# logv/sybil

Hardware: AMD Instinct MI355X
Metric: rows scanned/sec (1B-row x 32-int-col synthetic table, 3 ANDed int-range filters, group-by 2 cols, count/sum/avg/stddev of 2 cols) (higher is better)
Workload: dtype int64

## Files before the change

sybil_amd/csrc/planner.cpp:

```cpp
#include <math.h>
#include <stdlib.h>
#include <string.h>

#include <algorithm>

#include "engine.h"
#include "hll.h"
#include "re2lite.h"

namespace sybl {

static inline int64_t round_up(int64_t x, int64_t m) { return (x + m - 1) / m * m; }


struct HostFilterFold {
    bool has_range = false;
    int64_t lo = INT64_MIN, hi = INT64_MAX;
    std::vector<int64_t> neq;
    bool has_mask = false;
    std::vector<uint8_t> mask;
    std::vector<std::pair<int32_t, int32_t>> setp;
};

static void setup_buckets(int64_t info_min, int64_t info_max, int64_t hist_bucket, int64_t *bucket_size,
                          int64_t *num_buckets, int64_t *n_values) {
    int64_t size = info_max - info_min;
    int64_t nb = 1000;
    int64_t bs = size / nb;
    if (hist_bucket > 0) bs = hist_bucket;
    if (bs == 0) {
        if (size < 100) {
            bs = 1;
            nb = size;
        } else {
            bs = size / 100;
            nb = size / bs;
        }
    }
    nb += 1;
    *bucket_size = bs;
    *num_buckets = nb;
    *n_values = nb + 1;
}


static bool should_scan_block(const Table *t, const sybl_query_desc *d, int64_t b) {
    for (int i = 0; i < d->n_filters; i++) {
        const sybl_filter &f = d->filters[i];
        const Column *c = t->find(f.col);
        if (!c || c->type != SYBL_INT_VAL) continue;
        if (f.op != SYBL_OP_GT && f.op != SYBL_OP_LT && f.op != SYBL_OP_EQ) continue;
        if (c->blk_pop[(size_t)b] == 0) return false;
        int64_t mn = c->blk_min[(size_t)b], mx = c->blk_max[(size_t)b], v = f.int_value;
        if (f.op == SYBL_OP_GT && !(mn > v) && !(mx > v)) return false;
        if (f.op == SYBL_OP_LT && !(mn < v) && !(mx < v)) return false;
        if (f.op == SYBL_OP_EQ && (mn > v || mx < v)) return false;
    }
    return true;
}

constexpr int kEffWeightCol = -2;
constexpr int kRankColBase = -100;
static inline Column *slot_column(const Table *t, const Query *q, int ci) {
    if (ci <= kRankColBase) return t->cols[(size_t)(kRankColBase - ci)]->rank_col.get();
    return ci == kEffWeightCol ? q->eff_weight.get() : t->cols[(size_t)ci].get();
}

static bool fill_packed(Table *t, Query *q, const std::vector<int> &slot_col, FastPlan &FP, int nf, int ng, int na) {
    const ScanPlan &P = q->plan;
    if (env("SYBL_NO_PACKED")) return false;
    if (P.n_cells >= (1 << 24)) return false;
    for (int c = 0; c < nf; c++) {
        const __int128 umax = ((__int128)1 << (8 * FP.fwid[c])) - 1;
        const __int128 L = (__int128)FP.lo[c] - FP.fbase[c], H = (__int128)FP.hi[c] - FP.fbase[c];
        if (H < 0 || L > umax || L > H) {
            FP.plo[c] = 1;
            FP.phi[c] = 0;
        } else {
            FP.plo[c] = (uint32_t)(L < 0 ? 0 : L);
            FP.phi[c] = (uint32_t)(H > umax ? umax : H);
        }
        FP.npneq[c] = 0;
        for (int k = 0; k < FP.nneq[c]; k++) {
            const __int128 off = (__int128)FP.neq[c][k] - FP.fbase[c];
            if (off >= 0 && off <= umax) FP.pneq[c][FP.npneq[c]++] = (uint32_t)off;
        }
    }
    {
        double pass = 1.0;
        for (int c = 0; c < nf; c++) {
            const Column *col = nullptr;
            for (auto &cp : t->cols) {
                if (cp->d_data == (const void *)FP.fcol[c]) col = cp.get();
                if (cp->rank_col && cp->rank_col->d_data == (const void *)FP.fcol[c]) col = cp->rank_col.get();
            }
            if (FP.plo[c] > FP.phi[c]) {
                pass = 0.0;
            } else if (col && col->n_pop > 0 && col->exact_max >= col->vbase && !FP.fmask[c]) {
                const double top = (double)((__int128)col->exact_max - (__int128)col->vbase);
                const double hi = std::min((double)FP.phi[c], top), lo = (double)FP.plo[c];
                pass *= hi >= lo ? std::min(1.0, (hi - lo + 1.0) / (top + 1.0)) : 0.0;
            }
        }
        q->late_estimate = pass;
        FP.late = nf > 0 && pass < 0.005 ? 1 : 0;
        if (const char *e = env("SYBL_LATE_PATH")) FP.late = atoi(e) != 0;
    }
    for (int c = 0; c < ng; c++) FP.gdoff[c] = (uint32_t)((uint64_t)FP.gbase[c] - (uint64_t)FP.gmin[c]);
    for (int c = 0; c < na; c++) {
        const __int128 L = (__int128)FP.info_min[c] - FP.abase[c], H = (__int128)FP.max10[c] - FP.abase[c];
        const __int128 umax = ((__int128)1 << 32) - 1;
        if (H < 0 || L > umax || L > H) {
            FP.alo[c] = 1;
            FP.ahi[c] = 0;
        } else {
            FP.alo[c] = (uint32_t)(L < 0 ? 0 : L);
            FP.ahi[c] = (uint32_t)(H > umax ? umax : H);
        }
    }
    const double shave = 1.0 - 1.0 / (double)((int64_t)1 << 40);
    for (int c = 0; c < na; c++) {
        FP.adoff[c] = (uint32_t)((uint64_t)FP.abase[c] - (uint64_t)FP.hmin[c]);
        FP.pinv_bucket[c] = FP.bucket_size[c] ? (1.0 / (double)FP.bucket_size[c]) * shave : 0.0;
    }
    if (q->time_mode) {
        const SlotDesc &ts = P.slot[P.time_slot];
        const Column *tc = slot_column(t, q, slot_col[(size_t)P.time_slot]);
        if (P.tb_big_div || P.time_bucket >= ((int64_t)1 << 32)) return false;
        if (tc->n_pop > 0 && tc->exact_min < 0) return false;
        const __int128 t0 = (__int128)P.tb_min * P.time_bucket;
        const __int128 off = (__int128)ts.vbase - t0;
        const __int128 top = tc->n_pop > 0 ? (__int128)tc->exact_max - t0 : off;
        if (off < 0 || top >= ((__int128)1 << 32)) return false;
        FP.tdoff = (uint32_t)off;
        FP.pinv_time = (1.0 / (double)P.time_bucket) * shave;
    }
    return true;
}

#define FF_REJECT(...)                                                                                  \
    do {                                                                                                \
        if (env("SYBL_PLAN_TRACE")) fprintf(stderr, "fast path: rejected at planner.cpp:%d\n", __LINE__); \
        return __VA_ARGS__;                                                                             \
    } while (0)

static bool fill_fast_columns(Table *t, Query *q, const std::vector<int> &slot_col, FastPlan &FP, int *pnf, int *png,
                              int *pna, bool *any_max, bool *all_max, bool allow_gen, bool *gen, bool *packed = nullptr,
                              int max_groups = kFastTemplatedG, int max_aggs = kFastTemplatedA, bool part = false) {
    const ScanPlan &P = q->plan;
    memset(&FP, 0, sizeof(FP));
    int nf = 0, ng = 0, na = 0;
    *gen = false;
    bool any_packed = false, all_narrow = true;
    bool heavy = false;
    bool nul_needed = false;
    if (packed) *packed = false;
    for (size_t s = 0; s < slot_col.size(); s++) {
        const SlotDesc &sd = P.slot[s];
        if (sd.flags == 0 && q->pre_n_slots > 0) continue;
        const Column *c = slot_column(t, q, slot_col[s]);
        bool plain = c->type == SYBL_INT_VAL && !c->d_valid && !c->has_missing;
        any_packed = any_packed || c->packed();
        all_narrow = all_narrow && c->elem <= 4;
        if (!plain) {
            if (!allow_gen) FF_REJECT(false);
            uint32_t r2 = sd.flags & (kSlotFilter | kSlotGroup | kSlotAgg | kSlotTime);
            bool str_ok = c->type == SYBL_STR_VAL && (r2 == kSlotGroup || r2 == kSlotIdMask || r2 == (kSlotGroup | kSlotIdMask));
            if (c->type != SYBL_INT_VAL && !str_ok) FF_REJECT(false);
            *gen = true;
            if (c->d_valid || c->has_missing || (sd.flags & kSlotIdMask)) nul_needed = true;
        }
        uint32_t roles = sd.flags & (kSlotFilter | kSlotGroup | kSlotAgg);
        if (sd.flags & (kSlotSet | kSlotDict)) FF_REJECT(false);
        if ((sd.flags & kSlotNeq) && (!allow_gen || c->type != SYBL_INT_VAL)) FF_REJECT(false);
        if ((sd.flags & kSlotIdMask) && !allow_gen) FF_REJECT(false);
        if ((sd.flags & kSlotWeight) && (roles != 0 || (sd.flags & kSlotTime) || !allow_gen)) FF_REJECT(false);
// ... 1224 lines not shown
    std::vector<Segment> runs;
    bool quiet = false;

    int64_t max_lane_rows() const {
        if (q->dyn) return (int64_t)q->piece_cap * q->piece_tiles * kPackedRows;
        int64_t lane_rows = 0;
        for (int w = 0; w < q->n_wg; w++) {
            int64_t mine = 0;
            for (int32_t si = q->wg_seg_begin[(size_t)w]; si < q->wg_seg_begin[(size_t)w + 1]; si++)
                mine += (q->segs[(size_t)si].n + kPackedTileRows - 1) / kPackedTileRows * kPackedRows;
            lane_rows = std::max(lane_rows, mine);
        }
        return lane_rows;
    }

    void plan_count_packing() {
        FastPlan &FP = q->fplan;
        FP.cshift = 0;
        if (!q->fast || !q->fast_packed || q->fast_packed_n || q->part_hist || FP.nul || q->fast_na < 1 || env("SYBL_NO_CPACK")) return;
        if (q->fast_mode != kFastAvg && q->fast_mode != kFastAvgMax) return;
        const int64_t lane_rows = max_lane_rows();
        const unsigned __int128 slot_rows = (unsigned __int128)std::max<int64_t>(lane_rows, 1) * (unsigned __int128)(kWgThreads >> P.rep_shift);
        const Column *c = t->cols[(size_t)q->aggs[0].col].get();
        unsigned __int128 umax = c->elem >= 4 ? 0xFFFFFFFFull : c->elem == 2 ? 0xFFFFull : 0xFFull;
        if (c->n_pop > 0 && c->exact_max >= c->vbase) umax = std::min<unsigned __int128>(umax, (unsigned __int128)((__int128)c->exact_max - (__int128)c->vbase));
        auto bits = [](unsigned __int128 x) {
            int b = 0;
            while (x) b++, x >>= 1;
            return b;
        };
        const int sum_bits = std::max(1, bits(umax * slot_rows)), count_bits = bits(slot_rows);
        if (sum_bits + count_bits <= 64 && sum_bits < 63) FP.cshift = sum_bits;
        if (env("SYBL_PLAN_TRACE") && !quiet)
            fprintf(stderr, "count packing: cshift=%d sum_bits=%d count_bits=%d slot_rows=%lld\n", (int)FP.cshift, sum_bits, count_bits, (long long)slot_rows);
    }

    void plan_lean() {
        FastPlan &FP = q->fplan;
        FP.lean = 0;
        FP.lds_sum_fields = 0;
        if (!q->fast || !q->fast_packed || q->fast_packed_n || q->part_hist || FP.nul || q->fast_na < 1 || env("SYBL_NO_LEAN")) return;
        if (q->fast_mode != kFastMoments && q->fast_mode != kFastHist) return;
        const int na = q->fast_na;
        bool digits = !P.windowed, mul24 = true;
        for (size_t g = 0; g < q->groups.size() && digits; g++) {
            const int ci = q->groups[g].col;
            const Column *c = ci >= 0 ? t->cols[(size_t)ci].get() : nullptr;
            if (!c || c->type != SYBL_INT_VAL || c->n_pop <= 0 || q->groups[g].dict || q->groups[g].rank) {
                digits = false;
                break;
            }
            const __int128 lo = (__int128)c->exact_min - (__int128)FP.gmin[g], hi = (__int128)c->exact_max - (__int128)FP.gmin[g];
            digits = lo >= 0 && hi < (__int128)FP.gcard[g];
        }
        for (int a = 0; a < na; a++) {
            const Column *c = t->cols[(size_t)q->aggs[(size_t)a].col].get();
            if (FP.bucket_size[a] >= (1u << 24)) mul24 = false;
            if (c->n_pop > 0) {
                const __int128 lo = (__int128)c->exact_min - (__int128)FP.hmin[a], hi = (__int128)c->exact_max - (__int128)FP.hmin[a];
                if (lo < 0 || hi >= ((__int128)1 << 24)) mul24 = false;
            }
        }
        if (digits && mul24) FP.lean |= (int32_t)kLeanProved;
        if (q->fast_mode != kFastMoments) {
            if (env("SYBL_PLAN_TRACE") && !quiet) fprintf(stderr, "lean hist: proved=%d digits=%d mul24=%d\n", (FP.lean & (int32_t)kLeanProved) ? 1 : 0, (int)digits, (int)mul24);
            return;
        }
        const int words_now = P.n_sum_fields, words_lean = lean_sum_fields(na);
        bool shape = P.n_max_fields == 0 && P.n_sum_fields == 1 + 3 * na && FP.f_samples < 0 && FP.hist_lds == 0;
        for (int a = 0; a < na; a++) shape = shape && FP.f_sum[a] > 0 && FP.f_sb[a] > 0 && FP.f_sb2[a] > 0 && FP.f_cnt[a] < 0 && FP.f_pop[a] < 0 && FP.f_out[a] < 0;
        int rs = 0, cshift = 0;
        unsigned __int128 slot_rows = 0;
        uint64_t umax[kFastMaxA] = {0}, bmax[kFastMaxA] = {0};
        if (shape) {
            int64_t budget = kLdsBudgetBytes;
            if (!P.windowed)
                if (const char *e = env("SYBL_REP_BUDGET_KB")) budget = std::min<int64_t>(kLdsBudgetBytes, std::max<int64_t>(1, atoll(e)) * 1024);
            const int64_t bytes = (int64_t)words_lean * P.lds_cells * 8;
            while (rs < 6 && (bytes << (rs + 1)) <= budget) rs++;
            slot_rows = (unsigned __int128)std::max<int64_t>(max_lane_rows(), 1) * (unsigned __int128)(kWgThreads >> rs);
            for (int a = 0; a < na; a++) {
                const Column *c = t->cols[(size_t)q->aggs[(size_t)a].col].get();
                unsigned __int128 u = c->elem >= 4 ? 0xFFFFFFFFull : c->elem == 2 ? 0xFFFFull : 0xFFull;
                if (c->n_pop > 0 && c->exact_max >= c->vbase) u = std::min<unsigned __int128>(u, (unsigned __int128)((__int128)c->exact_max - (__int128)c->vbase));
                umax[a] = (uint64_t)u;
                bmax[a] = (uint64_t)std::max(FP.n_values[a] - 1, 0);
            }
            cshift = lean_moments_fit(na, umax, bmax, slot_rows);
        }
        if (cshift) {
            FP.lean |= (int32_t)kLeanMoments;
            FP.lds_sum_fields = words_lean;
            FP.cshift = cshift;
            P.rep_shift = rs;
            FP.rep_shift = rs;
            q->lds_bytes = ((size_t)words_lean * (size_t)P.lds_cells * 8) << rs;
        }
        if (env("SYBL_PLAN_TRACE") && !quiet) {
            fprintf(stderr, "lean moments: lean=%d proved=%d digits=%d mul24=%d cshift=%d count_bits=%d", cshift ? 1 : 0, (FP.lean & (int32_t)kLeanProved) ? 1 : 0,
                    (int)digits, (int)mul24, cshift, lean_bits(slot_rows));
            for (int a = 0; a < na && shape; a++)
                fprintf(stderr, " s%d_bits=%d b%d_bits=%d q%d_bits=%d", a, lean_bits((unsigned __int128)umax[a] * slot_rows), a,
                        lean_bits((unsigned __int128)bmax[a] * slot_rows), a, lean_bits((unsigned __int128)bmax[a] * bmax[a] * slot_rows));
            fprintf(stderr, " slot_rows=%lld tried_replicas=%d words=%d replicas=%d\n", (long long)slot_rows, 1 << rs, cshift ? words_lean : words_now,
                    1 << P.rep_shift);
        }
    }

    void plan_dynamic() {
        FastPlan &FP = q->fplan;
        const int32_t rep_shift0 = P.rep_shift, fp_rep_shift0 = FP.rep_shift;
        const size_t lds_bytes0 = q->lds_bytes;
        auto proofs = [&](bool dyn, bool silent) {
            P.rep_shift = rep_shift0;
            FP.rep_shift = fp_rep_shift0;
            q->lds_bytes = lds_bytes0;
// ... 520 lines not shown
```

sybil_amd/csrc/scan_fast.h:

```cpp
#pragma once
#include <hip/hip_runtime.h>
#include <stdint.h>

#include "plan.h"
#include "pieces.h"
#include "outlog.h"
#include "wg_header.h"

namespace sybl {

constexpr int kFastMaxF = 4, kFastMaxG = 4, kFastMaxA = 4;
constexpr int kFastTemplatedG = 2, kFastTemplatedA = 2;

enum FastMode : int {
    kFastAvg = 0,
    kFastAvgMax = 1,
    kFastMoments = 2,
    kFastHist = 3,
    kFastModes = 4,
};

struct FastPlan {
    const int64_t *fcol[kFastMaxF];
    const int64_t *gcol[kFastMaxG];
// ... 8 lines not shown
    int32_t n_values[kFastMaxA];
    int32_t f_sum[kFastMaxA], f_sb[kFastMaxA], f_sb2[kFastMaxA], m_max[kFastMaxA];
    int32_t m_nmin[kFastMaxA];
    int32_t ext_general;
    int64_t hist_agg_off[kFastMaxA];
    int64_t hist_off, hist_stride;
    int32_t n_cells, n_sum_fields, n_max_fields, rep_shift;
    const int64_t *tcol;
    int64_t time_bucket, tb_min;
    double inv_time_bucket;
    int32_t n_tb, tb_stride;
    int32_t windowed, lds_cells;
    int32_t hist_lds;
    int32_t lean;
    const uint32_t *fvalid[kFastMaxF], *gvalid[kFastMaxG], *avalid[kFastMaxA], *tvalid;
    int32_t gmissing[kFastMaxG], gvalues[kFastMaxG];
    int64_t gstride64[kFastMaxG], gmissing64[kFastMaxG], gvalues64[kFastMaxG], tb_stride64;
    const uint32_t *fmask[kFastMaxF];
    int32_t fmask_bits[kFastMaxF];
    int32_t nneq[kFastMaxF], npneq[kFastMaxF];
    int64_t neq[kFastMaxF][kMaxNeq];
    uint32_t pneq[kFastMaxF][kMaxNeq];
    int32_t f_cnt[kFastMaxA], f_pop[kFastMaxA], f_smp[kFastMaxA], f_out[kFastMaxA];
    int64_t info_min[kFastMaxA], max10[kFastMaxA];
    const int64_t *wcol;
    int32_t f_samples;
    int32_t cshift;
    int32_t fwid[kFastMaxF], gwid[kFastMaxG], awid[kFastMaxA], twid, wwid;
    int64_t fbase[kFastMaxF], gbase[kFastMaxG], abase[kFastMaxA], tbase, wbase;
    uint32_t plo[kFastMaxF], phi[kFastMaxF];
    uint32_t gdoff[kFastMaxG];
    uint32_t adoff[kFastMaxA];
    uint32_t tdoff;
    int32_t late;
    double pinv_bucket[kFastMaxA], pinv_time;
    uint32_t alo[kFastMaxA], ahi[kFastMaxA];
    int32_t nul;
    int32_t lds_sum_fields;
    const int32_t *wg_cell_base;
    const uint32_t *xvalid;
    int64_t *out_log;
    int64_t out_cap;
    int64_t *sum_out, *max_out, *ws_sum, *ws_max;
    const Segment *segs;
    const int32_t *wg_seg_begin;
    unsigned long long *wg_clock;
    int32_t dyn, n_pieces, piece_cap;
    const Piece *pieces;
    uint32_t *piece_queue;
    const uint32_t *fword;
    int32_t fshift[kFastMaxF], fbits[kFastMaxF];
    const uint32_t *kword;
    int32_t gshift[kFastMaxG], gbits[kFastMaxG], kashift, kabits;
};

hipError_t launch_scan_fast(const FastPlan &P, int nf, int ng, int na, int mode, bool time, bool gen, int n_wg,
                            size_t lds_bytes, hipStream_t st);

inline bool fast_plan_has_narrow(const FastPlan &P, bool aggs) {
    bool any = P.twid == 3 || P.wwid == 3 || (aggs && P.kword != nullptr);
    for (int c = 0; c < kFastMaxF; c++) any = any || P.fwid[c] == 3;
    for (int c = 0; c < kFastMaxG; c++) any = any || P.gwid[c] == 3;
    for (int c = 0; aggs && c < kFastMaxA; c++) any = any || P.awid[c] == 3;
    return any;
}

constexpr uint32_t kLeanMoments = 1u, kLeanProved = 2u;
constexpr int lean_sum_fields(int na) { return na + (na + 1) / 2 + na; }
constexpr int lean_bits(unsigned __int128 x) {
    int b = 0;
    while (x) b++, x >>= 1;
    return b;
}
constexpr int lean_moments_fit(int na, const uint64_t *umax, const uint64_t *bmax, unsigned __int128 slot_rows) {
    const unsigned __int128 one = 1;
    if (na < 1 || slot_rows < 1 || slot_rows >= (one << 63)) return 0;
    const int sum_bits = lean_bits((unsigned __int128)umax[0] * slot_rows) < 1 ? 1 : lean_bits((unsigned __int128)umax[0] * slot_rows);
    const int count_bits = lean_bits(slot_rows);
    if (!(sum_bits + count_bits <= 64 && sum_bits < 63)) return 0;
    const int shift = sum_bits < 32 ? 32 : sum_bits;
    if (shift + count_bits > 64) return 0;
    for (int c = 0; c < na; c++) {
        if (umax[c] >= (one << 32) || bmax[c] >= (one << 24)) return 0;
        if (c >= 1 && lean_bits((unsigned __int128)umax[c] * slot_rows) > 64) return 0;
        if (lean_bits((unsigned __int128)bmax[c] * bmax[c] * slot_rows) > 64) return 0;
        if ((unsigned __int128)bmax[c] * slot_rows >= (one << 32)) return 0;
    }
    return shift;
}
namespace lean_check {
constexpr uint64_t kU0[1] = {0}, kBfit[1] = {65535}, kBnot[1] = {65536};
static_assert(lean_moments_fit(1, kU0, kBfit, 65537) == 32, "sum(b) up to 2^32 - 1 fits a dword");
static_assert(lean_moments_fit(1, kU0, kBnot, 65536) == 0, "sum(b) of 2^32 does not");
constexpr uint64_t kU64[1] = {((uint64_t)1 << 23) - 1}, kU65[1] = {(uint64_t)1 << 23}, kB0[1] = {0};
static_assert(lean_moments_fit(1, kU64, kB0, (unsigned __int128)1 << 20) == 43, "64 bits of sum and count fit");
static_assert(lean_moments_fit(1, kU65, kB0, (unsigned __int128)1 << 20) == 0, "65 bits do not");
}

constexpr int kPartCells = 64;
constexpr int kPartCellBits = 6;
constexpr int kBucketBits = 10;
constexpr int kRecValueBits = 26;
constexpr int kMaxParts = 1024;
constexpr int kEmitMaxBins = 1024;
constexpr uint32_t kEmitChunk = 16;
constexpr uint32_t kEmitQueue = 32;
// ... 1072 lines not shown
```

sybil_amd/csrc/scan_packed.h:

```cpp
#pragma once
#include "narrow3.h"
#include "fword.h"
#include "scan_fast.h"

namespace sybl {

constexpr int kPackedRows = 4;
constexpr int kPackedTileRows = kWgThreads * kPackedRows;

hipError_t launch_scan_packed(const FastPlan &P, int nf, int ng, int na, int mode, bool time, int n_wg, size_t lds_bytes,
                              hipStream_t st);
hipError_t launch_emit_packed(const EmitPlan &E, int nf, int ng, int na, int n_wg, hipStream_t st);
hipError_t launch_count_packed_nf0(const EmitPlan &E, int ng, int n_wg, hipStream_t st);
hipError_t launch_count_packed_nf1(const EmitPlan &E, int ng, int n_wg, hipStream_t st);
hipError_t launch_count_packed_nf2(const EmitPlan &E, int ng, int n_wg, hipStream_t st);
hipError_t launch_count_packed_nf3(const EmitPlan &E, int ng, int n_wg, hipStream_t st);
hipError_t launch_count_packed_nf4(const EmitPlan &E, int ng, int n_wg, hipStream_t st);
hipError_t launch_emit_packed_nf0(const EmitPlan &E, int ng, int na, int n_wg, hipStream_t st);
hipError_t launch_emit_packed_nf1(const EmitPlan &E, int ng, int na, int n_wg, hipStream_t st);
hipError_t launch_emit_packed_nf2(const EmitPlan &E, int ng, int na, int n_wg, hipStream_t st);
hipError_t launch_emit_packed_nf3(const EmitPlan &E, int ng, int na, int n_wg, hipStream_t st);
hipError_t launch_emit_packed_nf4(const EmitPlan &E, int ng, int na, int n_wg, hipStream_t st);
hipError_t launch_scan_packed_nf0(const FastPlan &P, int ng, int na, int mode, bool time, int n_wg, size_t lds, hipStream_t st);
hipError_t launch_scan_packed_nf1(const FastPlan &P, int ng, int na, int mode, bool time, int n_wg, size_t lds, hipStream_t st);
// ... 122 lines not shown
__device__ __forceinline__ void packed_issue_ring(const FastPlan &P, const PackedBases<NF, NG, NA> &B, uint32_t r, uint32_t n,
                                                  PackedRaw<NF> &f, PackedRaw<NG> &g, PackedRaw<NA> &a, PackedRaw<1> &t) {
    const uint32_t r0 = __builtin_amdgcn_readfirstlane(r);
    const uint32_t lane_row = r - r0;
    const uint32_t rows = r0 < n ? (n - r0 < 64u * kPackedRows ? (n - r0 + kPackedRows - 1) & ~(uint32_t)(kPackedRows - 1) : 64u * kPackedRows) : 0u;
    const uint32_t base_row = rows ? r0 : 0u;
    auto issue = [&](const uint8_t *col, int width, pu32x4 &raw) {
        const uint32_t w = (uint32_t)width;
        const __amdgpu_buffer_rsrc_t rsrc =
            __builtin_amdgcn_make_buffer_rsrc((void *)(col + (size_t)(base_row * w)), 0, (int)(rows * w), (int)kBufferRsrcWord3);
        raw = __builtin_amdgcn_raw_buffer_load_b128(rsrc, (int)(__umul24(lane_row, w)), 0, 2);
    };
    if (TIME) issue(B.t, P.twid, t.v[0]);
#pragma unroll
    for (int c = 0; c < NF; c++) issue(B.f[c], P.fwid[c], f.v[c]);
#pragma unroll
    for (int c = 0; c < NG; c++) {
        if (G1) {
            const __amdgpu_buffer_rsrc_t rsrc = __builtin_amdgcn_make_buffer_rsrc((void *)(B.g[c] + (size_t)base_row), 0, (int)rows, (int)kBufferRsrcWord3);
            g.v[c].x = __builtin_amdgcn_raw_buffer_load_b32(rsrc, (int)lane_row, 0, 2);
        } else {
            issue(B.g[c], P.gwid[c], g.v[c]);
        }
    }
#pragma unroll
    for (int c = 0; c < NA; c++) issue(B.a[c], P.awid[c], a.v[c]);
}

constexpr int packed_depth(int) { return 1; }

template <int NF, int NG, int NA, bool TIME, bool G1, bool NUL, bool FRESH = false>
__device__ __forceinline__ void packed_decode_all(const FastPlan &P0, const PackedRaw<NF> &rf, const PackedRaw<NG> &rg,
                                                  const PackedRaw<NA> &ra, const PackedRaw<1> &rt, PackedTile<NF> &f,
                                                  PackedTile<NG> &g, PackedTile<NA> &a, PackedTile<1> &t, uint32_t bit0) {
    const FastPlan &P = plan_fresh<FRESH>(P0);
    if (NUL) {
        if (TIME) t.pop[0] = (rt.pw[0] >> bit0) & 0xFu;
#pragma unroll
        for (int c = 0; c < NF; c++) f.pop[c] = (rf.pw[c] >> bit0) & 0xFu;
#pragma unroll
        for (int c = 0; c < NG; c++) g.pop[c] = (rg.pw[c] >> bit0) & 0xFu;
#pragma unroll
        for (int c = 0; c < NA; c++) a.pop[c] = (ra.pw[c] >> bit0) & 0xFu;
    }
    if (TIME) packed_decode(P.twid, rt.v[0], t.u[0]);
#pragma unroll
    for (int c = 0; c < NF; c++) packed_decode(P.fwid[c], rf.v[c], f.u[c]);
#pragma unroll
    for (int c = 0; c < NG; c++) packed_decode(G1 ? 1 : P.gwid[c], rg.v[c], g.u[c]);
#pragma unroll
    for (int c = 0; c < NA; c++) packed_decode(P.awid[c], ra.v[c], a.u[c]);
}

template <bool M24 = false>
__device__ __forceinline__ uint32_t packed_udiv(uint32_t n, uint32_t d, double inv_lo) {
    uint32_t q = (uint32_t)((double)n * inv_lo);
    if (n - (M24 ? __umul24(q, d) : q * d) >= d) q += 1;
    return q;
}

template <int NF, int NG, int NA, int MODE, bool TIME, bool NUL, bool FRESH = false, bool OUT = false, bool MAX32 = false, bool LEAN = false,
          bool PROVED = false, bool COUNTED = false, bool DERIVED = false>
__device__ __forceinline__ void packed_row(const FastPlan &P0, const PackedTile<NF> &f, const PackedTile<NG> &g,
                                           const PackedTile<NA> &a, const PackedTile<1> &t, const int r, bool pass, int64_t *lds,
                                           const FastLds &L, uint32_t &matched, uint32_t &overflow, const uint32_t xpop = 0xFu) {
    static_assert(!LEAN || (MODE == kFastMoments && !NUL && !OUT && NA >= 1), "the lean layout is the plain moments body's");
    static_assert(!PROVED || (!NUL && !OUT), "proofs cover fully populated rows");
    static_assert(!DERIVED || (!NUL && !OUT), "only a row that counts in exactly one place can have its overflow derived");
    if (NUL) pass = pass & ((xpop >> r) & 1u);
#pragma unroll
    for (int c = 0; c < NF; c++) {
        const FastPlan &P = plan_fresh<FRESH>(P0);
        const uint32_t u = f.u[c][r];
        bool ok = (u >= P.plo[c]) & (u <= P.phi[c]);
        if (NUL) {
            if (P.fmask[c]) {
                const uint32_t id = u + (uint32_t)P.fbase[c];
                ok = id < (uint32_t)P.fmask_bits[c];
                if (ok) ok = (P.fmask[c][id >> 5] >> (id & 31)) & 1u;
            }
            for (int k = 0; k < P.npneq[c]; k++) ok = ok & (u != P.pneq[c][k]);
            ok = ok & ((f.pop[c] >> r) & 1u);
        }
        pass = pass & ok;
    }
    uint32_t cell = 0;
    bool inb = true;
#pragma unroll
    for (int c = 0; c < NG; c++) {
        const FastPlan &P = plan_fresh<FRESH>(P0);
        const uint32_t d = g.u[c][r] + P.gdoff[c];
        if (NUL) {
            const bool p = (g.pop[c] >> r) & 1u;
            inb = inb & (p ? d < (uint32_t)P.gvalues[c] : P.gmissing[c] >= 0);
            cell += p ? __umul24(d, (uint32_t)P.gstride[c]) : (uint32_t)P.gmissing[c];
        } else {
            if (!PROVED) inb = inb & (d < P.gcard[c]);
            cell += __umul24(d, (uint32_t)P.gstride[c]);
        }
    }
    bool live = pass;
    const FastPlan &P = plan_fresh<FRESH>(P0);
    if (TIME) {
        const uint32_t tb = packed_udiv(t.u[0][r] + P.tdoff, (uint32_t)P.time_bucket, P.pinv_time);
        if (NUL) {
            const bool tp = (t.pop[0] >> r) & 1u;
            live = live & tp;
            inb = inb & (tb < (uint32_t)P.n_tb || !tp);
        } else {
            inb = inb & (tb < (uint32_t)P.n_tb);
        }
        cell += __umul24(tb, (uint32_t)P.tb_stride);
    }
    const uint32_t ncell = L.tab_cells;
    const uint32_t lcell = cell - L.cell_base;
    inb = inb & (lcell < ncell);
    if (!COUNTED) matched += pass ? 1u : 0u;
    if (!DERIVED) overflow += (live & !inb) ? 1u : 0u;
    if (!(live & inb)) return;
    const uint32_t rs = (uint32_t)P.rep_shift;
    if (LEAN) {
        constexpr uint32_t kB = NA, kQ = NA + (NA + 1) / 2, kW = (uint32_t)lean_sum_fields(NA);
        const uint32_t chi = 1u << ((uint32_t)P.cshift - 32u);
        char *const lean_p = (char *)lds + __umul24((lcell << rs) + L.rep, kW * 8u);
        auto add = [&](uint32_t field, int64_t v) {
            __hip_atomic_fetch_add((int64_t *)(lean_p + field * 8u), v, __ATOMIC_RELAXED, __HIP_MEMORY_SCOPE_WORKGROUP);
        };
        uint32_t b[NA > 0 ? NA : 1];
#pragma unroll
        for (int c = 0; c < NA; c++) {
            const uint32_t u = a.u[c][r];
            add((uint32_t)c, (int64_t)(((uint64_t)(c == 0 ? chi : 0u) << 32) | u));
            b[c] = packed_udiv<PROVED>(u + P.adoff[c], P.bucket_size[c], P.pinv_bucket[c]);
            add(kQ + (uint32_t)c, (int64_t)(uint64_t)(uint32_t)__umul24(b[c], b[c]));
        }
#pragma unroll
        for (int j = 0; j < (NA + 1) / 2; j++)
            add(kB + (uint32_t)j, (int64_t)(((uint64_t)(2 * j + 1 < NA ? b[2 * j + 1 < NA ? 2 * j + 1 : 0] : 0u) << 32) | b[2 * j]));
        return;
    }
    char *const cell_p = (char *)lds + (((lcell << rs) + L.rep) << 3);
    const uint32_t fstep = (ncell << rs) << 3;
    auto add = [&](uint32_t field, int64_t v) {
        __hip_atomic_fetch_add((int64_t *)(cell_p + field * fstep), v, __ATOMIC_RELAXED, __HIP_MEMORY_SCOPE_WORKGROUP);
    };
    const uint32_t cshift = ((MODE == kFastAvg || MODE == kFastAvgMax) && !NUL && !OUT && NA > 0) ? (uint32_t)P.cshift : 0u;
    if (!cshift) add(0, 1);
#pragma unroll
    for (int c = 0; c < NA; c++) {
        const FastPlan &P = plan_fresh<FRESH>(P0);
        const uint32_t u = a.u[c][r];
        if (NUL) {
            if (!((a.pop[c] >> r) & 1u)) continue;
            if (P.f_pop[c] >= 0) add((uint32_t)P.f_pop[c], 1);
            if (P.f_cnt[c] >= 0) {
                if (u < P.alo[c] || u > P.ahi[c]) continue;
                add((uint32_t)P.f_cnt[c], 1);
            }
        }
        const int64_t x = (int64_t)((uint64_t)P.abase[c] + u);
        if (c == 0 && cshift) add((uint32_t)P.f_sum[0], (int64_t)(((uint64_t)1 << cshift) + u));
        else add((uint32_t)P.f_sum[c], x);
        if (MODE == kFastAvgMax) {
            if (MAX32) {
                __hip_atomic_fetch_max((uint32_t *)(cell_p + ((uint32_t)P.n_sum_fields + (uint32_t)P.m_max[c]) * fstep), u, __ATOMIC_RELAXED,
                                       __HIP_MEMORY_SCOPE_WORKGROUP);
            } else if (!P.ext_general) {
                int64_t *m = (int64_t *)(cell_p + ((uint32_t)P.n_sum_fields + (uint32_t)P.m_max[c]) * fstep);
                if (x > *m) __hip_atomic_fetch_max(m, x, __ATOMIC_RELAXED, __HIP_MEMORY_SCOPE_WORKGROUP);
            } else {
                if (P.m_max[c] >= 0) {
                    int64_t *m = (int64_t *)(cell_p + ((uint32_t)P.n_sum_fields + (uint32_t)P.m_max[c]) * fstep);
                    if (x > *m) __hip_atomic_fetch_max(m, x, __ATOMIC_RELAXED, __HIP_MEMORY_SCOPE_WORKGROUP);
                }
                if (P.m_nmin[c] >= 0) {
                    int64_t *m = (int64_t *)(cell_p + ((uint32_t)P.n_sum_fields + (uint32_t)P.m_nmin[c]) * fstep);
                    const int64_t nx = ~x;
                    if (nx > *m) __hip_atomic_fetch_max(m, nx, __ATOMIC_RELAXED, __HIP_MEMORY_SCOPE_WORKGROUP);
                }
            }
        }
        if (MODE == kFastMoments || MODE == kFastHist) {
            uint32_t b = packed_udiv<PROVED>(u + P.adoff[c], P.bucket_size[c], P.pinv_bucket[c]);
            if ((NUL || OUT) && b >= (uint32_t)P.n_values[c]) {
                if (P.f_out[c] >= 0) {
                    const unsigned __int128 sq = (unsigned __int128)((__int128)x * (__int128)x);
                    const uint32_t fo = (uint32_t)P.f_out[c];
                    add(fo, 1);
                    add(fo + 1, x);
                    add(fo + 2, (int64_t)(uint64_t)(sq & 0xFFFFFFFFu));
                    add(fo + 3, (int64_t)(uint64_t)((sq >> 32) & 0xFFFFFFFFu));
                    add(fo + 4, (int64_t)(uint64_t)((sq >> 64) & 0xFFFFFFFFu));
                    add(fo + 5, (int64_t)(uint64_t)(sq >> 96));
                    if (P.out_log) log_outlier(P.out_log, P.out_cap, (int64_t)cell, c, x);
                } else {
                    overflow += 1;
                }
                b = (uint32_t)P.n_values[c] - 1;
            }
            if (MODE == kFastMoments) {
                add((uint32_t)P.f_sb[c], (int64_t)(uint64_t)b);
                add((uint32_t)P.f_sb2[c], (int64_t)(uint64_t)(uint32_t)__umul24(b, b));
            } else if (P.hist_lds) {
                __hip_atomic_fetch_add(L.hist32 + lcell * (uint32_t)P.hist_stride + (uint32_t)P.hist_agg_off[c] + b, 1u,
                                       __ATOMIC_RELAXED, __HIP_MEMORY_SCOPE_WORKGROUP);
            } else {
                __hip_atomic_fetch_add(P.sum_out + P.hist_off + (int64_t)cell * P.hist_stride + P.hist_agg_off[c] + b,
                                       (int64_t)1, __ATOMIC_RELAXED, __HIP_MEMORY_SCOPE_AGENT);
            }
        }
    }
}

template <int NF, int NG, int NA, int MODE, bool TIME, bool FRESH, bool COUNTED, int LEANV, class PASS>
__device__ __forceinline__ void packed_plain_tile(const FastPlan &P, const PackedTile<NF> &f, const PackedTile<NG> &g, const PackedTile<NA> &a,
                                                  const PackedTile<1> &t, PASS pass, int64_t *lds, const FastLds &L, const bool max32,
                                                  uint32_t &matched, uint32_t &overflow) {
    constexpr bool kLean = (LEANV & kLeanMoments) != 0, kProved = (LEANV & kLeanProved) != 0;
    if (MODE == kFastAvgMax && max32) {
#pragma unroll
        for (int k = 0; k < kPackedRows; k++)
            packed_row<NF, NG, NA, MODE, TIME, false, FRESH, false, true, false, false, COUNTED, true>(P, f, g, a, t, k, pass(k), lds, L, matched, overflow);
    } else {
#pragma unroll
        for (int k = 0; k < kPackedRows; k++)
            packed_row<NF, NG, NA, MODE, TIME, false, FRESH, false, false, kLean, kProved, COUNTED, true>(P, f, g, a, t, k, pass(k), lds, L, matched, overflow);
    }
}

constexpr int64_t kPackedChunkRows = (int64_t)1 << 28;

#ifndef SYBL_PACKED_LATE
#define SYBL_PACKED_LATE 1
#endif
constexpr bool kPackedLate = SYBL_PACKED_LATE != 0;
#ifndef SYBL_PACKED_LATE_BRANCH
#define SYBL_PACKED_LATE_BRANCH 1
#endif
constexpr bool kPackedLateBranch = SYBL_PACKED_LATE_BRANCH != 0;

#ifndef SYBL_PACKED_WAVES_PER_EU
#define SYBL_PACKED_WAVES_PER_EU 4
#endif

static_assert(kPackedTileRows == kPieceTileRows, "pieces.h counts k_scan_packed's tiles");
struct DynTile {
    int64_t R;
    uint32_t rows;
};
constexpr uint32_t kNoTicket = 0xFFFFFFFFu;

static_assert(sizeof(Piece) == 16 && offsetof(Piece, start) == 0 && offsetof(Piece, n) == 8, "enter_piece reads a piece as four dwords");
struct DynCursor {
    const FastPlan &P;
    uint32_t *ring;
    uint32_t k = 0;
    int64_t R = 0;
    uint32_t left = 0;
    bool done = false;
    uint32_t pend = kNoTicket, drawn = 0;
    bool pend_ok = false;
    bool want_draw = false;

    __device__ __forceinline__ DynCursor(const FastPlan &P_, uint32_t *ring_) : P(P_), ring(ring_) {
        if (threadIdx.x == 0) {
            draw();
            ring[0] = pend_ok ? pend : kNoTicket;
            draw();
        }
        __syncthreads();
    }
    __device__ __forceinline__ void draw() {
        pend_ok = drawn < (uint32_t)P.piece_cap;
        if (pend_ok) {
            pend = __builtin_amdgcn_atomic_inc32(P.piece_queue, 0xFFFFFFFFu, __ATOMIC_RELAXED, "agent");
            drawn++;
        }
    }
    __device__ __forceinline__ void enter_piece() {
// ... 3 lines not shown
            if (ahead >= (uint32_t)P.n_pieces) drawn = (uint32_t)P.piece_cap;
            ring[(k + 1) & 3u] = ahead;
            want_draw = true;
        }
        __syncthreads();
        const uint32_t ticket = __builtin_amdgcn_readfirstlane(ring[k & 3u]);
        k++;
        const bool have = ticket < (uint32_t)P.n_pieces;
        typedef const __attribute__((address_space(4))) pu32x4 *piece_words;
        const pu32x4 pc = *(piece_words)(uintptr_t)(P.pieces + (have ? ticket : 0u));
        R = (int64_t)(((uint64_t)pc.y << 32) | pc.x);
        left = have ? pc.z : 0u;
        done = !have;
    }
    __device__ __forceinline__ void draw_ahead() {
        if (threadIdx.x == 0 && want_draw) {
            draw();
            want_draw = false;
        }
    }
    __device__ __forceinline__ DynTile next() {
        if (left == 0 && !done) enter_piece();
        DynTile T;
        T.R = ((int64_t)__builtin_amdgcn_readfirstlane((int)(R >> 32)) << 32) | (uint32_t)__builtin_amdgcn_readfirstlane((int)(uint32_t)R);
        left = __builtin_amdgcn_readfirstlane(left);
        T.rows = left < (uint32_t)kPackedTileRows ? left : (uint32_t)kPackedTileRows;
        R = T.R + kPackedTileRows;
        left -= T.rows;
        return T;
    }
};

template <int NF, int NG, int NA, int MODE, bool TIME, bool G1, int LEANV, bool FW, bool KW>
__device__ __forceinline__ void packed_scan_dyn(const FastPlan &P, int64_t *lds, const FastLds &L, const bool max32, uint32_t &matched,
                                                uint32_t &overflow) {
    static_assert(!FW || NF >= kFwordMinFields, "a filter word holds at least two columns");
    static_assert(kFwordMaxFields == kFastMaxF, "one field per filter column of a FastPlan");
    static_assert(!KW || (!TIME && !G1 && NF >= 1 && NG >= 1 && NA >= 1), "a key word holds the keys and aggregation 0 of the late loop");
    static_assert(!KW || kPackedLate, "a key word is read by the late loop");
    static_assert(!KW || NG + 1 <= kFwordMaxFields, "one field per key column and one for aggregation 0");
    __shared__ uint32_t ring[4];
    const uint32_t tid = threadIdx.x;
    const uint32_t wave_row = __builtin_amdgcn_readfirstlane((tid & ~63u) * kPackedRows);
    const uint32_t lane_row = (tid & 63u) * kPackedRows;
    DynCursor cur(P, ring);
    PackedRaw<NF> rf;
    PackedRaw<NG> rg;
    PackedRaw<NA> ra;
    PackedRaw<1> rt;
    PackedTile<NF> f;
    PackedTile<NG> g;
    PackedTile<NA> a;
    PackedTile<1> t;
    auto issue = [&](const void *col, int width, const DynTile &T, bool wanted, pu32x4 &raw, bool one_dword) {
        const uint32_t rows = wanted && T.rows > wave_row
                                  ? (T.rows - wave_row < 64u * kPackedRows ? (T.rows - wave_row + kPackedRows - 1) & ~(uint32_t)(kPackedRows - 1) : 64u * kPackedRows)
                                  : 0u;
        const int64_t base = rows ? T.R + wave_row : 0;
        const uint32_t w = (uint32_t)width;
        const __amdgpu_buffer_rsrc_t rsrc =
            __builtin_amdgcn_make_buffer_rsrc((void *)((const uint8_t *)col + (size_t)base * w), 0, (int)(rows * w), (int)kBufferRsrcWord3);
        if (one_dword) raw.x = __builtin_amdgcn_raw_buffer_load_b32(rsrc, (int)lane_row, 0, 2);
        else raw = __builtin_amdgcn_raw_buffer_load_b128(rsrc, (int)(__umul24(lane_row, w)), 0, 2);
    };
    auto issue_filters = [&](const DynTile &T) {
        if constexpr (FW) {
            issue(P.fword, 4, T, true, rf.v[0], false);
        } else {
#pragma unroll
            for (int c = 0; c < NF; c++) issue(P.fcol[c], P.fwid[c], T, true, rf.v[c], false);
        }
    };
    auto decode_filters = [&]() {
        if constexpr (FW) {
            const uint32_t wd[kPackedRows] = {rf.v[0].x, rf.v[0].y, rf.v[0].z, rf.v[0].w};
#pragma unroll
            for (int c = 0; c < NF; c++) {
#pragma unroll
                for (int k = 0; k < kPackedRows; k++) f.u[c][k] = __builtin_amdgcn_ubfe(wd[k], (uint32_t)P.fshift[c], (uint32_t)P.fbits[c]);
            }
        } else {
#pragma unroll
            for (int c = 0; c < NF; c++) packed_decode(P.fwid[c], rf.v[c], f.u[c]);
        }
    };
    auto issue_rest = [&](const DynTile &T, bool wanted) {
        if (TIME) issue(P.tcol, P.twid, T, wanted, rt.v[0], false);
        if constexpr (KW) {
            issue(P.kword, 4, T, wanted, ra.v[0], false);
        } else {
#pragma unroll
            for (int c = 0; c < NG; c++) issue(P.gcol[c], G1 ? 1 : P.gwid[c], T, wanted, rg.v[c], G1);
        }
#pragma unroll
        for (int c = KW ? 1 : 0; c < NA; c++) issue(P.acol[c], P.awid[c], T, wanted, ra.v[c], false);
    };
    auto decode_rest = [&]() {
        if (TIME) packed_decode(P.twid, rt.v[0], t.u[0]);
        if constexpr (KW) {
            const uint32_t wd[kPackedRows] = {ra.v[0].x, ra.v[0].y, ra.v[0].z, ra.v[0].w};
#pragma unroll
            for (int c = 0; c < NG; c++) {
#pragma unroll
                for (int k = 0; k < kPackedRows; k++) g.u[c][k] = __builtin_amdgcn_ubfe(wd[k], (uint32_t)P.gshift[c], (uint32_t)P.gbits[c]);
            }
#pragma unroll
            for (int k = 0; k < kPackedRows; k++) a.u[0][k] = __builtin_amdgcn_ubfe(wd[k], (uint32_t)P.kashift, (uint32_t)P.kabits);
        } else {
#pragma unroll
            for (int c = 0; c < NG; c++) packed_decode(G1 ? 1 : P.gwid[c], rg.v[c], g.u[c]);
        }
#pragma unroll
        for (int c = KW ? 1 : 0; c < NA; c++) packed_decode(P.awid[c], ra.v[c], a.u[c]);
    };
    auto lane_left = [&](const DynTile &T) -> uint32_t { return T.rows > tid * kPackedRows ? T.rows - tid * kPackedRows : 0u; };
    if (kPackedLate && NF > 0 && NG + NA + (TIME ? 1 : 0) > 0) {
        PackedTile<0> f0;
        auto filter_bits = [&](const DynTile &T) -> uint32_t {
            decode_filters();
            const uint32_t left = lane_left(T);
            uint32_t bits = 0;
#pragma unroll
            for (int k = 0; k < kPackedRows; k++) {
                bool pass = (uint32_t)k < left;
#pragma unroll
                for (int c = 0; c < NF; c++) pass = pass & (f.u[c][k] >= P.plo[c]) & (f.u[c][k] <= P.phi[c]);
                bits |= pass ? 1u << k : 0u;
            }
            return bits;
        };
        DynTile T0 = cur.next();
        issue_filters(T0);
        uint32_t bits = filter_bits(T0);
        DynTile T1 = cur.next();
        issue_rest(T0, __builtin_amdgcn_ballot_w64(bits != 0) != 0);
        issue_filters(T1);
        cur.draw_ahead();
        while (T0.rows) {
            decode_rest();
            const uint32_t next_bits = filter_bits(T1);
            const DynTile T2 = cur.next();
            if (kPackedLateBranch) {
                if (__builtin_amdgcn_ballot_w64(next_bits != 0) != 0) issue_rest(T1, true);
            } else {
                issue_rest(T1, __builtin_amdgcn_ballot_w64(next_bits != 0) != 0);
            }
            issue_filters(T2);
            cur.draw_ahead();
            matched += (uint32_t)__builtin_popcount(bits);
            packed_plain_tile<0, NG, NA, MODE, TIME, false, true, LEANV>(P, f0, g, a, t, [&](int k) -> bool { return (bits >> k) & 1u; }, lds, L, max32,
                                                                         matched, overflow);
            bits = next_bits;
            T0 = T1;
            T1 = T2;
        }
        return;
    }
    DynTile T0 = cur.next();
    issue_filters(T0);
    issue_rest(T0, true);
    cur.draw_ahead();
    while (T0.rows) {
        decode_filters();
        decode_rest();
        const DynTile T1 = cur.next();
        issue_filters(T1);
        issue_rest(T1, true);
        cur.draw_ahead();
        const uint32_t left = lane_left(T0);
        if (NF == 0) matched += left < (uint32_t)kPackedRows ? left : (uint32_t)kPackedRows;
        packed_plain_tile<NF, NG, NA, MODE, TIME, false, NF == 0, LEANV>(P, f, g, a, t, [&](int k) { return (uint32_t)k < left; }, lds, L, max32,
                                                                        matched, overflow);
        T0 = T1;
    }
}
template <int NF, int NG, int NA, int MODE, bool TIME, bool G1, bool NUL, int RING = 0, int LEANV = 0, bool DYN = false, bool FW = false,
          bool KW = false>
__global__ __launch_bounds__(kWgThreads, SYBL_PACKED_WAVES_PER_EU) void k_scan_packed(const FastPlan P) {
    static_assert(LEANV == 0 || !NUL, "the NUL kernels mix row bodies: no proofs");
    static_assert(!DYN || (!NUL && RING == 0), "dynamic dealing is the plain kernels'");
    static_assert(!FW || (DYN && NF >= kFwordMinFields), "filter words are the dynamic loops', for two filter columns and more");
    static_assert(!KW || (DYN && !TIME && !G1 && NG >= 1 && NA >= 1 && FW == (NF >= kFwordMinFields) && NF >= 1),
                  "key words are the dynamic late loop's: keys and an aggregation, one filter column or a filter word");
    static_assert(!(LEANV & kLeanMoments) || (MODE == kFastMoments && NA >= 1), "the lean layout is moments mode's");
    static_assert(!(LEANV & kLeanProved) || MODE == kFastMoments || MODE == kFastHist, "the proved bodies are the bucket modes'");
    extern __shared__ int64_t lds[];
    const uint32_t tid = threadIdx.x;
    constexpr bool kMax32 = MODE == kFastAvgMax && !NUL;
    constexpr bool lean_layout = (LEANV & kLeanMoments) != 0;
    const FastLds L = fast_begin<MODE>(P, lds, kMax32 && !P.ext_general, lean_layout);

    uint32_t matched = 0, overflow = 0;
    const uint64_t clock_in = P.wg_clock ? wall_clock64() : 0;
    if constexpr (DYN) packed_scan_dyn<NF, NG, NA, MODE, TIME, G1, LEANV, FW, KW>(P, lds, L, kMax32 && !P.ext_general, matched, overflow);
    const int s0 = DYN ? 0 : P.wg_seg_begin[blockIdx.x], s1 = DYN ? 0 : P.wg_seg_begin[blockIdx.x + 1];
    for (int si = s0; si < s1; si++) {
        const Segment seg = P.segs[si];
        for (int64_t c0 = 0; c0 < seg.n; c0 += kPackedChunkRows) {
            const int64_t first = seg.start + c0;
            const uint32_t n = (uint32_t)(seg.n - c0 < kPackedChunkRows ? seg.n - c0 : kPackedChunkRows);
            PackedBases<NF, NG, NA> B;
#pragma unroll
            for (int c = 0; c < NF; c++) B.f[c] = (const uint8_t *)P.fcol[c] + first * P.fwid[c];
#pragma unroll
            for (int c = 0; c < NG; c++) B.g[c] = (const uint8_t *)P.gcol[c] + first * P.gwid[c];
#pragma unroll
            for (int c = 0; c < NA; c++) B.a[c] = (const uint8_t *)P.acol[c] + first * P.awid[c];
            B.t = TIME ? (const uint8_t *)P.tcol + first * P.twid : nullptr;
            B.first = first;

            PackedTile<NF> f;
            PackedTile<NG> g;
            PackedTile<NA> a;
            PackedTile<1> t;
            constexpr bool FRESH = RING == 4;
            constexpr int D = NUL ? 1 : (RING > 0 && RING < 4 ? RING : packed_depth(NF + NG + NA + (TIME ? 1 : 0)));
            if (D > 1) {
                PackedRaw<NF> rf[D];
                PackedRaw<NG> rg[D];
                PackedRaw<NA> ra[D];
                PackedRaw<1> rt[D];
                const uint32_t n_tiles = (n + kPackedTileRows - 1) / kPackedTileRows;
                const uint32_t r_first = tid * kPackedRows;
#pragma unroll
                for (int d = 0; d < D; d++) {
// ... 712 lines not shown
```

Before: 527.4 billion.

## Replace proved-path bucket division with magic multiply and fold group offsets

On the proved lean path, the bucket index is now computed with a precomputed multiply-high-and-shift magic constant. This replaces the double-precision reciprocal multiply followed by a correction step. Group-key offsets are folded at plan time into a single constant cell base, so the per-column add and the cell_base subtract disappear. Several plan scalars (bit widths, chi, zero, kfold) are also pinned into VGPRs to avoid repeated scalar-to-vector moves in the unrolled row loop. New proof conditions tighten when the proved path applies, which could push some queries back onto the slower path.

```diff
diff --git a/sybil_amd/csrc/planner.cpp b/sybil_amd/csrc/planner.cpp
--- a/sybil_amd/csrc/planner.cpp
+++ b/sybil_amd/csrc/planner.cpp
@@ -5,6 +5,7 @@
 #include <algorithm>
 
 #include "engine.h"
+#include "udiv_magic.h"
 #include "hll.h"
 #include "re2lite.h"
 
@@ -106,7 +107,11 @@
         FP.late = nf > 0 && pass < 0.005 ? 1 : 0;
         if (const char *e = env("SYBL_LATE_PATH")) FP.late = atoi(e) != 0;
     }
-    for (int c = 0; c < ng; c++) FP.gdoff[c] = (uint32_t)((uint64_t)FP.gbase[c] - (uint64_t)FP.gmin[c]);
+    FP.kfold = 0;
+    for (int c = 0; c < ng; c++) {
+        FP.gdoff[c] = (uint32_t)((uint64_t)FP.gbase[c] - (uint64_t)FP.gmin[c]);
+        FP.kfold += FP.gdoff[c] * (uint32_t)FP.gstride[c];
+    }
     for (int c = 0; c < na; c++) {
         const __int128 L = (__int128)FP.info_min[c] - FP.abase[c], H = (__int128)FP.max10[c] - FP.abase[c];
         const __int128 umax = ((__int128)1 << 32) - 1;
@@ -122,6 +127,10 @@
     for (int c = 0; c < na; c++) {
         FP.adoff[c] = (uint32_t)((uint64_t)FP.abase[c] - (uint64_t)FP.hmin[c]);
         FP.pinv_bucket[c] = FP.bucket_size[c] ? (1.0 / (double)FP.bucket_size[c]) * shave : 0.0;
+        const UdivMagic m = udiv_magic(FP.bucket_size[c]);
+        FP.qmul[c] = m.mul;
+        FP.qshift[c] = m.shift;
+        FP.qoff2[c] = FP.adoff[c] << 1;
     }
     if (q->time_mode) {
         const SlotDesc &ts = P.slot[P.time_slot];
@@ -1452,16 +1461,23 @@
             }
             const __int128 lo = (__int128)c->exact_min - (__int128)FP.gmin[g], hi = (__int128)c->exact_max - (__int128)FP.gmin[g];
             digits = lo >= 0 && hi < (__int128)FP.gcard[g];
+            if ((__int128)c->exact_max - (__int128)FP.gbase[g] >= ((__int128)1 << 24) || (uint32_t)FP.gstride[g] >= (1u << 24)) digits = false;
         }
         for (int a = 0; a < na; a++) {
             const Column *c = t->cols[(size_t)q->aggs[(size_t)a].col].get();
-            if (FP.bucket_size[a] >= (1u << 24)) mul24 = false;
+            if (FP.bucket_size[a] < 1 || FP.bucket_size[a] >= (1u << 24)) mul24 = false;
             if (c->n_pop > 0) {
                 const __int128 lo = (__int128)c->exact_min - (__int128)FP.hmin[a], hi = (__int128)c->exact_max - (__int128)FP.hmin[a];
                 if (lo < 0 || hi >= ((__int128)1 << 24)) mul24 = false;
             }
         }
         if (digits && mul24) FP.lean |= (int32_t)kLeanProved;
+        if ((FP.lean & (int32_t)kLeanProved) && env("SYBL_PLAN_TRACE") && !quiet) {
+            fprintf(stderr, "quotient:");
+            for (int a = 0; a < na; a++)
+                fprintf(stderr, " a%d d=%u mul=%u shift=%u off2=%u", a, (unsigned)FP.bucket_size[a], (unsigned)FP.qmul[a], (unsigned)FP.qshift[a], (unsigned)FP.qoff2[a]);
+            fprintf(stderr, " kfold=%u\n", (unsigned)FP.kfold);
+        }
         if (q->fast_mode != kFastMoments) {
             if (env("SYBL_PLAN_TRACE") && !quiet) fprintf(stderr, "lean hist: proved=%d digits=%d mul24=%d\n", (FP.lean & (int32_t)kLeanProved) ? 1 : 0, (int)digits, (int)mul24);
             return;
diff --git a/sybil_amd/csrc/scan_fast.h b/sybil_amd/csrc/scan_fast.h
--- a/sybil_amd/csrc/scan_fast.h
+++ b/sybil_amd/csrc/scan_fast.h
@@ -84,6 +84,8 @@
     int32_t fshift[kFastMaxF], fbits[kFastMaxF];
     const uint32_t *kword;
     int32_t gshift[kFastMaxG], gbits[kFastMaxG], kashift, kabits;
+    uint32_t qmul[kFastMaxA], qshift[kFastMaxA], qoff2[kFastMaxA];
+    uint32_t kfold;
 };
 
 hipError_t launch_scan_fast(const FastPlan &P, int nf, int ng, int na, int mode, bool time, bool gen, int n_wg,
diff --git a/sybil_amd/csrc/scan_packed.h b/sybil_amd/csrc/scan_packed.h
--- a/sybil_amd/csrc/scan_packed.h
+++ b/sybil_amd/csrc/scan_packed.h
@@ -198,18 +198,28 @@
     for (int c = 0; c < NA; c++) packed_decode(P.awid[c], ra.v[c], a.u[c]);
 }
 
-template <bool M24 = false>
 __device__ __forceinline__ uint32_t packed_udiv(uint32_t n, uint32_t d, double inv_lo) {
     uint32_t q = (uint32_t)((double)n * inv_lo);
-    if (n - (M24 ? __umul24(q, d) : q * d) >= d) q += 1;
+    if (n - q * d >= d) q += 1;
     return q;
 }
+
+template <bool PROVED>
+__device__ __forceinline__ uint32_t packed_bucket(const FastPlan &P, const int c, const uint32_t u) {
+    if (PROVED) return __umulhi((u << 1) + P.qoff2[c], P.qmul[c]) >> P.qshift[c];
+    return packed_udiv(u + P.adoff[c], P.bucket_size[c], P.pinv_bucket[c]);
+}
+
+struct PackedRowRegs {
+    uint32_t kfold, chi, zero;
+};
 
 template <int NF, int NG, int NA, int MODE, bool TIME, bool NUL, bool FRESH = false, bool OUT = false, bool MAX32 = false, bool LEAN = false,
           bool PROVED = false, bool COUNTED = false, bool DERIVED = false>
 __device__ __forceinline__ void packed_row(const FastPlan &P0, const PackedTile<NF> &f, const PackedTile<NG> &g,
                                            const PackedTile<NA> &a, const PackedTile<1> &t, const int r, bool pass, int64_t *lds,
-                                           const FastLds &L, uint32_t &matched, uint32_t &overflow, const uint32_t xpop = 0xFu) {
+                                           const FastLds &L, uint32_t &matched, uint32_t &overflow, const uint32_t xpop = 0xFu,
+                                           const PackedRowRegs *X = nullptr) {
     static_assert(!LEAN || (MODE == kFastMoments && !NUL && !OUT && NA >= 1), "the lean layout is the plain moments body's");
     static_assert(!PROVED || (!NUL && !OUT), "proofs cover fully populated rows");
     static_assert(!DERIVED || (!NUL && !OUT), "only a row that counts in exactly one place can have its overflow derived");
@@ -230,12 +240,12 @@
         }
         pass = pass & ok;
     }
-    uint32_t cell = 0;
+    uint32_t cell = PROVED ? (X ? X->kfold : plan_fresh<FRESH>(P0).kfold - L.cell_base) : 0u;
     bool inb = true;
 #pragma unroll
     for (int c = 0; c < NG; c++) {
         const FastPlan &P = plan_fresh<FRESH>(P0);
-        const uint32_t d = g.u[c][r] + P.gdoff[c];
+        const uint32_t d = PROVED ? g.u[c][r] : g.u[c][r] + P.gdoff[c];
         if (NUL) {
             const bool p = (g.pop[c] >> r) & 1u;
             inb = inb & (p ? d < (uint32_t)P.gvalues[c] : P.gmissing[c] >= 0);
@@ -259,7 +269,7 @@
         cell += __umul24(tb, (uint32_t)P.tb_stride);
     }
     const uint32_t ncell = L.tab_cells;
-    const uint32_t lcell = cell - L.cell_base;
+    const uint32_t lcell = PROVED ? cell : cell - L.cell_base;
     inb = inb & (lcell < ncell);
     if (!COUNTED) matched += pass ? 1u : 0u;
     if (!DERIVED) overflow += (live & !inb) ? 1u : 0u;
@@ -267,7 +277,7 @@
     const uint32_t rs = (uint32_t)P.rep_shift;
     if (LEAN) {
         constexpr uint32_t kB = NA, kQ = NA + (NA + 1) / 2, kW = (uint32_t)lean_sum_fields(NA);
-        const uint32_t chi = 1u << ((uint32_t)P.cshift - 32u);
+        const uint32_t chi = X ? X->chi : 1u << ((uint32_t)P.cshift - 32u), zero = X ? X->zero : 0u;
         char *const lean_p = (char *)lds + __umul24((lcell << rs) + L.rep, kW * 8u);
         auto add = [&](uint32_t field, int64_t v) {
             __hip_atomic_fetch_add((int64_t *)(lean_p + field * 8u), v, __ATOMIC_RELAXED, __HIP_MEMORY_SCOPE_WORKGROUP);
@@ -276,13 +286,13 @@
 #pragma unroll
         for (int c = 0; c < NA; c++) {
             const uint32_t u = a.u[c][r];
-            add((uint32_t)c, (int64_t)(((uint64_t)(c == 0 ? chi : 0u) << 32) | u));
-            b[c] = packed_udiv<PROVED>(u + P.adoff[c], P.bucket_size[c], P.pinv_bucket[c]);
-            add(kQ + (uint32_t)c, (int64_t)(uint64_t)(uint32_t)__umul24(b[c], b[c]));
+            add((uint32_t)c, (int64_t)(((uint64_t)(c == 0 ? chi : zero) << 32) | u));
+            b[c] = packed_bucket<PROVED>(P, c, u);
+            add(kQ + (uint32_t)c, (int64_t)(((uint64_t)zero << 32) | (uint32_t)__umul24(b[c], b[c])));
         }
 #pragma unroll
         for (int j = 0; j < (NA + 1) / 2; j++)
-            add(kB + (uint32_t)j, (int64_t)(((uint64_t)(2 * j + 1 < NA ? b[2 * j + 1 < NA ? 2 * j + 1 : 0] : 0u) << 32) | b[2 * j]));
+            add(kB + (uint32_t)j, (int64_t)(((uint64_t)(2 * j + 1 < NA ? b[2 * j + 1 < NA ? 2 * j + 1 : 0] : zero) << 32) | b[2 * j]));
         return;
     }
     char *const cell_p = (char *)lds + (((lcell << rs) + L.rep) << 3);
@@ -327,7 +337,7 @@
             }
         }
         if (MODE == kFastMoments || MODE == kFastHist) {
-            uint32_t b = packed_udiv<PROVED>(u + P.adoff[c], P.bucket_size[c], P.pinv_bucket[c]);
+            uint32_t b = packed_bucket<PROVED>(P, c, u);
             if ((NUL || OUT) && b >= (uint32_t)P.n_values[c]) {
                 if (P.f_out[c] >= 0) {
                     const unsigned __int128 sq = (unsigned __int128)((__int128)x * (__int128)x);
@@ -351,7 +361,7 @@
                 __hip_atomic_fetch_add(L.hist32 + lcell * (uint32_t)P.hist_stride + (uint32_t)P.hist_agg_off[c] + b, 1u,
                                        __ATOMIC_RELAXED, __HIP_MEMORY_SCOPE_WORKGROUP);
             } else {
-                __hip_atomic_fetch_add(P.sum_out + P.hist_off + (int64_t)cell * P.hist_stride + P.hist_agg_off[c] + b,
+                __hip_atomic_fetch_add(P.sum_out + P.hist_off + (int64_t)(PROVED ? cell + L.cell_base : cell) * P.hist_stride + P.hist_agg_off[c] + b,
                                        (int64_t)1, __ATOMIC_RELAXED, __HIP_MEMORY_SCOPE_AGENT);
             }
         }
@@ -361,7 +371,7 @@
 template <int NF, int NG, int NA, int MODE, bool TIME, bool FRESH, bool COUNTED, int LEANV, class PASS>
 __device__ __forceinline__ void packed_plain_tile(const FastPlan &P, const PackedTile<NF> &f, const PackedTile<NG> &g, const PackedTile<NA> &a,
                                                   const PackedTile<1> &t, PASS pass, int64_t *lds, const FastLds &L, const bool max32,
-                                                  uint32_t &matched, uint32_t &overflow) {
+                                                  uint32_t &matched, uint32_t &overflow, const PackedRowRegs *X = nullptr) {
     constexpr bool kLean = (LEANV & kLeanMoments) != 0, kProved = (LEANV & kLeanProved) != 0;
     if (MODE == kFastAvgMax && max32) {
 #pragma unroll
@@ -370,7 +380,8 @@
     } else {
 #pragma unroll
         for (int k = 0; k < kPackedRows; k++)
-            packed_row<NF, NG, NA, MODE, TIME, false, FRESH, false, false, kLean, kProved, COUNTED, true>(P, f, g, a, t, k, pass(k), lds, L, matched, overflow);
+            packed_row<NF, NG, NA, MODE, TIME, false, FRESH, false, false, kLean, kProved, COUNTED, true>(P, f, g, a, t, k, pass(k), lds, L, matched, overflow,
+                                                                                                          0xFu, X);
     }
 }
 
@@ -480,6 +491,30 @@
     PackedTile<NG> g;
     PackedTile<NA> a;
     PackedTile<1> t;
+    auto pinned = [](uint32_t x) -> uint32_t {
+        asm volatile("" : "+v"(x));
+        return x;
+    };
+    uint32_t fbits_v[NF > 0 ? NF : 1] = {}, gbits_v[NG > 0 ? NG : 1] = {}, kabits_v = 0;
+    if constexpr (FW) {
+#pragma unroll
+        for (int c = 0; c < NF; c++) fbits_v[c] = pinned((uint32_t)P.fbits[c]);
+    }
+    if constexpr (KW) {
+#pragma unroll
+        for (int c = 0; c < NG; c++) gbits_v[c] = pinned((uint32_t)P.gbits[c]);
+        kabits_v = pinned((uint32_t)P.kabits);
+    }
+    constexpr bool kRowRegs = (LEANV & kLeanProved) != 0;
+    PackedRowRegs regs = {0, 0, 0};
+    if constexpr (kRowRegs) {
+        regs.kfold = pinned(P.kfold - L.cell_base);
+        if constexpr ((LEANV & kLeanMoments) != 0) {
+            regs.chi = pinned(1u << ((uint32_t)P.cshift - 32u));
+            regs.zero = pinned(0u);
+        }
+    }
+    const PackedRowRegs *const X = kRowRegs ? &regs : nullptr;
     auto issue = [&](const void *col, int width, const DynTile &T, bool wanted, pu32x4 &raw, bool one_dword) {
         const uint32_t rows = wanted && T.rows > wave_row
                                   ? (T.rows - wave_row < 64u * kPackedRows ? (T.rows - wave_row + kPackedRows - 1) & ~(uint32_t)(kPackedRows - 1) : 64u * kPackedRows)
@@ -505,7 +540,7 @@
 #pragma unroll
             for (int c = 0; c < NF; c++) {
 #pragma unroll
-                for (int k = 0; k < kPackedRows; k++) f.u[c][k] = __builtin_amdgcn_ubfe(wd[k], (uint32_t)P.fshift[c], (uint32_t)P.fbits[c]);
+                for (int k = 0; k < kPackedRows; k++) f.u[c][k] = __builtin_amdgcn_ubfe(wd[k], (uint32_t)P.fshift[c], fbits_v[c]);
             }
         } else {
 #pragma unroll
@@ -530,10 +565,10 @@
 #pragma unroll
             for (int c = 0; c < NG; c++) {
 #pragma unroll
-                for (int k = 0; k < kPackedRows; k++) g.u[c][k] = __builtin_amdgcn_ubfe(wd[k], (uint32_t)P.gshift[c], (uint32_t)P.gbits[c]);
-            }
-#pragma unroll
-            for (int k = 0; k < kPackedRows; k++) a.u[0][k] = __builtin_amdgcn_ubfe(wd[k], (uint32_t)P.kashift, (uint32_t)P.kabits);
+                for (int k = 0; k < kPackedRows; k++) g.u[c][k] = __builtin_amdgcn_ubfe(wd[k], (uint32_t)P.gshift[c], gbits_v[c]);
+            }
+#pragma unroll
+            for (int k = 0; k < kPackedRows; k++) a.u[0][k] = __builtin_amdgcn_ubfe(wd[k], (uint32_t)P.kashift, kabits_v);
         } else {
 #pragma unroll
             for (int c = 0; c < NG; c++) packed_decode(G1 ? 1 : P.gwid[c], rg.v[c], g.u[c]);
@@ -577,7 +612,7 @@
             cur.draw_ahead();
             matched += (uint32_t)__builtin_popcount(bits);
             packed_plain_tile<0, NG, NA, MODE, TIME, false, true, LEANV>(P, f0, g, a, t, [&](int k) -> bool { return (bits >> k) & 1u; }, lds, L, max32,
-                                                                         matched, overflow);
+                                                                         matched, overflow, X);
             bits = next_bits;
             T0 = T1;
             T1 = T2;
@@ -598,7 +633,7 @@
         const uint32_t left = lane_left(T0);
         if (NF == 0) matched += left < (uint32_t)kPackedRows ? left : (uint32_t)kPackedRows;
         packed_plain_tile<NF, NG, NA, MODE, TIME, false, NF == 0, LEANV>(P, f, g, a, t, [&](int k) { return (uint32_t)k < left; }, lds, L, max32,
-                                                                        matched, overflow);
+                                                                        matched, overflow, X);
         T0 = T1;
     }
 }
diff --git a/sybil_amd/csrc/udiv_magic.h b/sybil_amd/csrc/udiv_magic.h
--- /dev/null
+++ b/sybil_amd/csrc/udiv_magic.h
@@ -0,0 +1,38 @@
+#pragma once
+#include <cstdint>
+
+namespace sybl {
+
+constexpr uint32_t kUdivMagicLimit = 1u << 24;
+
+struct UdivMagic {
+    uint32_t mul, shift;
+};
+
+constexpr UdivMagic udiv_magic(uint32_t d) {
+    if (d < 1 || d >= kUdivMagicLimit) return UdivMagic{0, 0};
+    uint32_t s = 0;
+    while ((d >> (s + 1)) != 0) s++;
+    const uint64_t p = (uint64_t)1 << (31 + s);
+    return UdivMagic{(uint32_t)((p + d - 1) / d), s};
+}
+
+constexpr uint32_t udiv_magic_apply(uint32_t n, UdivMagic m) { return (uint32_t)(((uint64_t)(n << 1) * m.mul) >> 32) >> m.shift; }
+
+namespace udiv_magic_check {
+constexpr bool at(uint32_t n, uint32_t d) { return n >= kUdivMagicLimit || udiv_magic_apply(n, udiv_magic(d)) == n / d; }
+constexpr bool edges(uint32_t d) {
+    const uint32_t top = kUdivMagicLimit - 1, kmax = top / d, kmid = kmax / 2 + 1;
+    return udiv_magic(d).mul > (1u << 30) && udiv_magic(d).mul <= (1u << 31) && at(top, d) && at(0, d) && at(d - 1, d) && at(d, d) &&
+           at(kmid * d - 1, d) && at(kmid * d, d) && at(kmax * d - 1, d) && at(kmax * d, d);
+}
+static_assert(udiv_magic(1).mul == (1u << 31) && udiv_magic(1).shift == 0, "d = 1: q = (2 n * 2^31) >> 32 = n");
+static_assert(udiv_magic(1000).shift == 9 && udiv_magic(1000).mul == 1099511628u, "ceil(2^40 / 1000)");
+static_assert(edges(1) && edges(2) && edges(3), "the smallest bucket sizes");
+static_assert(edges(999) && edges(1000) && edges(4096), "bucket sizes of the benchmark's kind, a power of two");
+static_assert(edges((1u << 23) - 1) && edges(1u << 23) && edges((1u << 23) + 1), "around the last power of two");
+static_assert(edges((1u << 24) - 2) && edges((1u << 24) - 1), "the largest bucket sizes");
+static_assert(udiv_magic(0).mul == 0 && udiv_magic(1u << 24).mul == 0, "outside the proof: no constants");
+}
+
+}
```

New measurement: 577.2 billion (median of 6 runs). 9.4% higher.
